# JzHuai0108/sim3opt

Measured on AMD Instinct MI355X. Metric: LM iterations/s, higher is better.
Workload: dtype f64

## Files before the change

include/sim3opt.h:

```cpp
#ifndef SIM3OPT_H
#define SIM3OPT_H

#include <stdint.h>

#ifdef __cplusplus
extern "C" {
#endif

typedef struct sim3opt_graph sim3opt_graph;

enum {
  SIM3OPT_OK = 0,
  SIM3OPT_ERR_ARG = -1,
  SIM3OPT_ERR_STATE = -2,
  SIM3OPT_ERR_NO_DEVICE = -3,
  SIM3OPT_ERR_HIP = -4,
  SIM3OPT_ERR_IO = -5,
  SIM3OPT_ERR_COMM = -6
};

enum { SIM3OPT_KERNEL_NONE = 0, SIM3OPT_KERNEL_HUBER = 1, SIM3OPT_KERNEL_PSEUDO_HUBER = 2,
       SIM3OPT_KERNEL_CAUCHY = 3, SIM3OPT_KERNEL_GEMAN_MCCLURE = 4, SIM3OPT_KERNEL_WELSCH = 5,
       SIM3OPT_KERNEL_FAIR = 6, SIM3OPT_KERNEL_TUKEY = 7, SIM3OPT_KERNEL_SATURATED = 8,
       SIM3OPT_KERNEL_DCS = 9 };

typedef struct sim3opt_options {
  double tau;
  double user_lambda_init;
  double good_step_lower;
  double good_step_upper;
  int32_t max_trials;
  double fd_delta;
  double exp_eps;
  int32_t small_rot_half;
  int32_t fix_small_angle_b;
  int32_t dof_mask;
  int32_t pcg_max_iters;
  double pcg_rel_tol;
  int32_t pcg_check_every;
  int32_t pcg_graph;
  int32_t preconditioner;
  int32_t chain_segment;
  int32_t device;
  int32_t verbose;
  int32_t time_kernels;
  int32_t linear_solver;
  int32_t amg_cycle[4];
  int32_t amg_passes[3];
  int32_t amg_additive;
  int32_t amg_fp32;
  int32_t amg_pivot;
  int32_t amg_coarsest;
  int32_t adaptive_prec;
  int32_t row_order;
  int32_t halo_exchange;
  int32_t span_grid;
  int32_t force_collectives;
  int32_t amg_shard_rows;
  int32_t amg_virtual_ranks;
  int32_t pcg_batch;
  double amg_omega;
  double amg_over[2];
  int64_t direct_max_pairs;
  int32_t debug_full_arrays;
  int32_t jacobians;
  int32_t algorithm;
  int32_t dl_max_trials;
  double dl_delta_init;
  double dl_lambda_init;
  double dl_lambda_factor;
  double cov_workspace_mb;
  int32_t cov_solver;
  double cov_rel_tol;
} sim3opt_options;

enum {
  SIM3OPT_ALGORITHM_LM = 0,
  SIM3OPT_ALGORITHM_GAUSS_NEWTON = 1,
  SIM3OPT_ALGORITHM_DOGLEG = 2
};

enum {
  SIM3OPT_STEP_UNDEFINED = 0,
  SIM3OPT_STEP_SD = 1,
  SIM3OPT_STEP_GN = 2,
  SIM3OPT_STEP_DL = 3
};

typedef struct sim3opt_tr_stats {
  double delta_before;
  double delta_after;
  double alpha;
  double norm_sd;
  double norm_gn;
  double norm_dl;
  int32_t step;
  int32_t was_pd;
} sim3opt_tr_stats;

typedef struct sim3opt_iter_stats {
  double chi2_before;
  double chi2_after;
  double lambda;
  double rho;
  int32_t trials;
  int32_t pcg_iters;
  double pcg_rel_res;
  double ms_linearize;
  double ms_solve;
  double ms_update;
  int32_t pcg_capped;
  int32_t reserved_;
} sim3opt_iter_stats;

typedef struct sim3opt_kernel_times {
  double ms_spmv;      int64_t n_spmv;
  double ms_pcg_vec;   int64_t n_pcg_vec;
  double ms_linearize; int64_t n_linearize;
  double ms_chi2;      int64_t n_chi2;
  double ms_update;    int64_t n_update;
  double ms_replicated_levels; int64_t n_replicated_visits;
  int64_t n_batches; int64_t n_batched_solves;
} sim3opt_kernel_times;

typedef struct sim3opt_comm_times {
  double ms_allreduce;  int64_t n_allreduce;  int64_t bytes_allreduce;
// ... 235 lines not shown
```

sim3opt_amd/csrc/amg_kernels.hpp:

```cpp
#pragma once

__global__ __launch_bounds__(WG) void k_amg_adjoint(int nb, const int32_t* __restrict__ row2v,
                                                    const Sim3* __restrict__ states,
                                                    double* __restrict__ P) {
  for (int i = blockIdx.x * WG + threadIdx.x; i < nb; i += gridDim.x * WG) {
  const Sim3 S = load_sim3(states + row2v[i]);
  double R[9];
  sim3::R_from_quat(S.q, R);
  double A[49];
#pragma unroll
  for (int k = 0; k < 49; ++k) A[k] = 0.0;
  const double t0 = S.t[0], t1 = S.t[1], t2 = S.t[2];
#pragma unroll
  for (int c = 0; c < 3; ++c) {
    const double v0 = R[c], v1 = R[3 + c], v2 = R[6 + c];
    A[0 + 7 * c] = v0;
    A[1 + 7 * c] = v1;
    A[2 + 7 * c] = v2;
    A[3 + 7 * c] = t1 * v2 - t2 * v1;
    A[4 + 7 * c] = t2 * v0 - t0 * v2;
    A[5 + 7 * c] = t0 * v1 - t1 * v0;
    A[3 + 7 * (3 + c)] = S.s * v0;
    A[4 + 7 * (3 + c)] = S.s * v1;
    A[5 + 7 * (3 + c)] = S.s * v2;
// ... 461 lines not shown
  for (int m = 0; m < PB; ++m) {
    double cm[4], rm[4];
#pragma unroll
    for (int a = 0; a < 4; ++a) cm[a] = colk[ty + 16 * a][m];
#pragma unroll
    for (int b = 0; b < 4; ++b) rm[b] = rowk[m][tx + 16 * b];
#pragma unroll
    for (int a = 0; a < 4; ++a)
#pragma unroll
      for (int b = 0; b < 4; ++b) v[a][b] -= cm[a] * rm[b];
  }
#pragma unroll
  for (int a = 0; a < 4; ++a) {
    const int i = i0 + ty + 16 * a, ip = i - k0;
    const bool ik = ip >= 0 && ip < PB;
#pragma unroll
    for (int b = 0; b < 4; ++b) {
      const int jl = tx + 16 * b, j = j0 + jl;
      if (i < n && j < n) B[(size_t)i * n + j] = ik ? rowk[ip][jl] : v[a][b];
    }
  }
}

template <int K>
__global__ __launch_bounds__(WG) void k_amg_dense_apply(int n, const double* __restrict__ Ainv,
                                                        const double* __restrict__ r,
                                                        double* __restrict__ x, int64_t as, int64_t vs) {
  const int lane = threadIdx.x & 63;
  if (gridDim.y > 1) {
    const size_t s0 = (size_t)blockIdx.y * K;
    Ainv += s0 * as;
    r += s0 * vs;
    x += s0 * vs;
  }
  for (int i = blockIdx.x * 4 + (threadIdx.x >> 6); i < n; i += gridDim.x * 4) {
#pragma unroll
    for (int s = 0; s < K; ++s) {
      const double* row = Ainv + (size_t)s * as + (size_t)i * n;
      const double* rs = r + (size_t)s * vs;
      double a0 = 0.0, a1 = 0.0, a2 = 0.0, a3 = 0.0;
      int j = lane;
      for (; j + 192 < n; j += 256) {
        const double m0 = row[j], m1 = row[j + 64], m2 = row[j + 128], m3 = row[j + 192];
        a0 += m0 * rs[j]; a1 += m1 * rs[j + 64]; a2 += m2 * rs[j + 128]; a3 += m3 * rs[j + 192];
      }
      for (; j < n; j += 64) a0 += row[j] * rs[j];
      double acc = (a0 + a1) + (a2 + a3);
      acc = wave_sum(acc);
      if (lane == 0) x[(size_t)s * vs + i] = acc;
    }
  }
}

__global__ __launch_bounds__(WG) void k_to_f32(size_t n, const double* __restrict__ src,
                                               float* __restrict__ dst) {
  for (size_t i = (size_t)blockIdx.x * WG + threadIdx.x; i < n; i += (size_t)gridDim.x * WG)
    dst[f32_pair_index((int64_t)(i / 49), (int)(i % 49))] = (float)src[i];
}
```

sim3opt_amd/csrc/capi.cpp:

```cpp
#include <algorithm>
#include <cmath>
#include <cstdlib>
#include <chrono>
#include <cstring>
#include <memory>
#include <new>
#include <string>
#include <vector>

#include "../../include/sim3opt.h"
#include "../../include/sim3opt_bench.h"
#include "amg.hpp"
#include "col_plan.hpp"
#include "comm.hpp"
#include "devmem.hpp"
#include "direct.hpp"
#include "engine.hpp"
#include "graph.hpp"
#include "robust.hpp"
#include "sim3_jac.hpp"

using namespace sim3opt;

struct sim3opt_graph {
// ... 106 lines not shown

int sim3opt_version(void) { return 130; }

void sim3opt_options_default(sim3opt_options* o) {
  if (!o) return;
  o->tau = 1e-5;
  o->user_lambda_init = 0.0;
  o->good_step_lower = 1.0 / 3.0;
  o->good_step_upper = 2.0 / 3.0;
  o->max_trials = 10;
  o->fd_delta = 1e-9;
  o->exp_eps = 1e-5;
  o->small_rot_half = 0;
  o->fix_small_angle_b = 0;
  o->dof_mask = 127;
  o->pcg_max_iters = 0;
  o->pcg_rel_tol = 1e-10;
  o->pcg_check_every = 16;
  o->pcg_graph = 1;
  o->preconditioner = -1;
  o->chain_segment = 256;
  o->device = -1;
  o->verbose = 0;
  o->time_kernels = 0;
  o->linear_solver = -1;
  for (int32_t& v : o->amg_cycle) v = 0;
  for (int32_t& v : o->amg_passes) v = 0;
  o->amg_additive = 0;
  o->amg_fp32 = 1;
  o->amg_pivot = 14;
  o->amg_coarsest = 256;
  o->adaptive_prec = 1;
  o->row_order = -1;
  o->halo_exchange = 1;
  o->span_grid = 0;
  o->force_collectives = 0;
  o->amg_shard_rows = 4096;
  o->amg_virtual_ranks = 0;
  o->pcg_batch = 0;
  o->amg_omega = 0.9;
  o->amg_over[0] = 1.8;
  o->amg_over[1] = 1.6;
  o->direct_max_pairs = 0;
  o->debug_full_arrays = 0;
  o->jacobians = 0;
  o->algorithm = SIM3OPT_ALGORITHM_LM;
  o->dl_max_trials = 100;
  o->dl_delta_init = 1e4;
  o->dl_lambda_init = 1e-7;
  o->dl_lambda_factor = 10.0;
  o->cov_workspace_mb = 256.0;
  o->cov_solver = 0;
  o->cov_rel_tol = 1e-8;
}

static void apply_env_overrides(sim3opt_options& o) {
  auto digits = [](const char* ev, int32_t* dst, int n, int lo, int hi) {
    int last = 0;
    const int len = (int)std::strlen(ev);
    for (int l = 0; l < n; ++l) {
      if (l < len && ev[l] - '0' >= lo && ev[l] - '0' <= hi) last = ev[l] - '0';
      dst[l] = last;
    }
  };
  if (const char* ev = std::getenv("SIM3OPT_AMG_CYCLE")) digits(ev, o.amg_cycle, 4, 1, 3);
  if (const char* ev = std::getenv("SIM3OPT_AMG_PASSES")) digits(ev, o.amg_passes, 3, 1, 6);
  if (const char* ev = std::getenv("SIM3OPT_AMG_ADDITIVE")) o.amg_additive = std::atoi(ev) != 0;
  if (const char* ev = std::getenv("SIM3OPT_AMG_FP32")) o.amg_fp32 = std::atoi(ev) != 0;
  if (const char* ev = std::getenv("SIM3OPT_AMG_PIVOT")) o.amg_pivot = std::atoi(ev);
  if (const char* ev = std::getenv("SIM3OPT_AMG_COARSEST")) o.amg_coarsest = std::atoi(ev);
  if (const char* ev = std::getenv("SIM3OPT_ADAPTIVE_PREC")) o.adaptive_prec = std::atoi(ev) != 0;
  if (const char* ev = std::getenv("SIM3OPT_ROW_ORDER")) o.row_order = std::string(ev) == "bfs" ? 1 : 0;
  if (std::getenv("SIM3OPT_NO_HALO")) o.halo_exchange = 0;
  if (const char* ev = std::getenv("SIM3OPT_SPAN_GRID")) o.span_grid = std::atoi(ev);
  if (const char* ev = std::getenv("SIM3OPT_FORCE_COMM")) o.force_collectives = ev[0] == '1';
  if (const char* ev = std::getenv("SIM3OPT_AMG_SHARD_ROWS")) o.amg_shard_rows = std::atoi(ev);
  if (const char* ev = std::getenv("SIM3OPT_AMG_VIRTUAL_RANKS")) o.amg_virtual_ranks = std::atoi(ev);
  if (const char* ev = std::getenv("SIM3OPT_PCG_BATCH")) o.pcg_batch = std::atoi(ev);
  if (const char* ev = std::getenv("SIM3OPT_AMG_OMEGA")) o.amg_omega = std::atof(ev);
  if (const char* ev = std::getenv("SIM3OPT_AMG_OVER")) {
    o.amg_over[0] = o.amg_over[1] = std::atof(ev);
    if (const char* c = std::strchr(ev, ',')) o.amg_over[1] = std::atof(c + 1);
  }
  if (const char* ev = std::getenv("SIM3OPT_DIRECT_MAX_PAIRS")) o.direct_max_pairs = std::atoll(ev);
  if (const char* ev = std::getenv("SIM3OPT_DEBUG_FULL_ARRAYS")) o.debug_full_arrays = std::atoi(ev) != 0;
  if (const char* ev = std::getenv("SIM3OPT_COV_WORKSPACE_MB"))
    if (std::atof(ev) > 0.0) o.cov_workspace_mb = std::atof(ev);
  if (const char* ev = std::getenv("SIM3OPT_COV_SOLVER"))
    if (std::atoi(ev) >= 0 && std::atoi(ev) <= 2) o.cov_solver = std::atoi(ev);
  if (const char* ev = std::getenv("SIM3OPT_COV_REL_TOL"))
    if (std::atof(ev) > 0.0 && std::atof(ev) <= 1e-2) o.cov_rel_tol = std::atof(ev);
}

sim3opt_graph* sim3opt_create(void) {
  sim3opt_graph* g = new (std::nothrow) sim3opt_graph();
  if (g) {
    sim3opt_options_default(&g->opt);
    sim3opt::handle_count(+1);
  }
  return g;
}

void sim3opt_destroy(sim3opt_graph* g) {
  if (!g) return;
  delete g;
  if (sim3opt::handle_count(-1) == 0) sim3opt::dev_cache_release();
}

void sim3opt_release_device_cache(void) { sim3opt::dev_cache_release(); }

int sim3opt_set_options(sim3opt_graph* g, const sim3opt_options* o) {
  if (!g || !o) return fail(g, SIM3OPT_ERR_ARG, "set_options: null argument");
  if (!(o->fd_delta > 0) || !(o->exp_eps > 0) || o->max_trials < 1 || !(o->pcg_rel_tol >= 0) ||
      !(o->tau > 0) || o->pcg_check_every < 0 || o->amg_virtual_ranks < 0 || o->pcg_batch < 0 ||
      o->direct_max_pairs < 0 || !(o->amg_omega > 0) || !(o->amg_over[0] > 0) || !(o->amg_over[1] > 0))
    return fail(g, SIM3OPT_ERR_ARG, "set_options: value out of range");
  if (o->jacobians != 0 && o->jacobians != 1)
    return fail(g, SIM3OPT_ERR_ARG, "set_options: jacobians must be 0 (numeric) or 1 (analytic)");
  if (o->algorithm < SIM3OPT_ALGORITHM_LM || o->algorithm > SIM3OPT_ALGORITHM_DOGLEG)
    return fail(g, SIM3OPT_ERR_ARG, "set_options: algorithm must be 0 (LM), 1 (Gauss-Newton) or 2 (dogleg)");
  {
    auto pos = [](double v) { return std::isfinite(v) && v > 0.0; };
// ... 946 lines not shown
```

sim3opt_amd/csrc/engine_amg.hip:

```cpp
#include "engine_impl.hpp"

#include <cassert>

namespace sim3opt {

#include "spmv_kernel.hpp"
#include "amg_kernels.hpp"

int Engine::amg_init(const Structure& s, bool automatic, std::string& err) {
  (void)err;
  amg_omega = std::max(0.1, std::min(0.95, opt.amg_omega));
  amg_additive = opt.amg_additive != 0;
  {
    const bool partitioned = part_world() >= 2;
    int last = 0;
    for (int l = 1; l <= AMG_MAX_LEVELS; ++l) {
      const int o = l <= 4 ? opt.amg_cycle[l - 1] : 0;
      if (o >= 1 && o <= 3) last = o;
      amg_visits[l] = last > 0 ? last : (partitioned ? (l <= 1 ? 1 : 2) : (l <= 1 ? 2 : 3));
    }
    amg_visits[0] = 1;
  }
  amg_fp32 = opt.amg_fp32 != 0;
  adaptive_prec = opt.adaptive_prec != 0 && automatic;
  amg_pivot = opt.amg_pivot >= 28 ? 28 : 14;
  for (int l = 0; l <= AMG_MAX_LEVELS; ++l)
    amg_over_l[l] = std::max(0.5, std::min(3.0, l == 0 ? opt.amg_over[0] : opt.amg_over[1]));
  std::string why;
  AmgBuildOptions bo;
  bo.max_coarsest = opt.amg_coarsest;
  for (int k = 0; k < 3; ++k) bo.passes[k] = opt.amg_passes[k];
  std::vector<int32_t> vbegin;
  bo.world = part_world();
  bo.shard_rows = std::max(1, opt.amg_shard_rows);
  if (comm.world > 1) {
    bo.row_begin = row_begin.data();
  } else if (bo.world > 1) {
    vbegin.resize(bo.world + 1);
    partition_rows_equal(nb, bo.world, vbegin.data());
    bo.row_begin = vbegin.data();
  }
  if (!build_amg_hierarchy(nb, s.rowptr.data(), s.colidx.data(), amg_host, why, bo)) {
    if (opt.verbose) std::fprintf(stderr, "sim3opt: no multigrid hierarchy (%s)\n", why.c_str());
    amg_host.clear();
    return SIM3OPT_OK;
  }
  if (automatic && (double)amg_host[1].nnzb > 0.3 * (double)amg_host[0].nnzb) {
    if (opt.verbose)
      std::fprintf(stderr, "sim3opt: the graph coarsens like an expander (level-1 blocks %.2f of level 0): block-Jacobi\n",
                   (double)amg_host[1].nnzb / (double)amg_host[0].nnzb);
    amg_host.clear();
    return SIM3OPT_OK;
  }
  use_amg = true;
  return SIM3OPT_OK;
}

int Engine::amg_bind(const Structure& s, std::string& err) {
  std::vector<AmgLevelHost>& H = amg_host;
  const int nl = (int)H.size();
  amg.assign(nl, AmgLevel());
  int rc = SIM3OPT_OK;
#define AMGCHK(call) do { rc = (call); if (rc) return rc; } while (0)
  AmgLevel& L0 = amg[0];
  L0.nb = nb; L0.nnzb = nnzb;
  L0.rowptr = d_rowptr; L0.colidx = d_colidx; L0.wrow = d_wrow; L0.span_grid = span_grid;
  L0.vals = d_vals; L0.Minv = d_Minv; L0.r = d_r; L0.x = d_z;
  int64_t padded = 0;
  (void)allgather_equal_plan(offs.data(), comm.world, nullptr, &padded);
  AMGCHK(amg_alloc(d_az, std::max<size_t>((size_t)n, (size_t)padded), err));
  AMGCHK(amg_alloc(d_P, (size_t)49 * nb, err));
  AMGCHK(amg_up(d_row2v, s.row2vertex, err));
  L0.t = d_az;
  L0.lo = r0; L0.hi = r1;
  const int64_t shard_rows = std::max(1, opt.amg_shard_rows);
  rep_level = 1;
  while (rep_level < nl - 1 && H[rep_level].nb > shard_rows && !H[rep_level].row_begin.empty() &&
         H[rep_level].respects_owner)
// ... 159 lines not shown
    const int pb = pivot_rows(k0), pbn = k0 + pb < nd ? pivot_rows(k0 + pb) : 0;
    if (pb == 28)
      hipLaunchKernelGGL((k_amg_dense_gj_step<28>), gt, dim3(WG), 0, stream, nd, k0, (const double*)src,
                         dst, (const double*)pin, pout, pbn, sc);
    else if (pb == 14)
      hipLaunchKernelGGL((k_amg_dense_gj_step<14>), gt, dim3(WG), 0, stream, nd, k0, (const double*)src,
                         dst, (const double*)pin, pout, pbn, sc);
    else
      hipLaunchKernelGGL((k_amg_dense_gj_step<7>), gt, dim3(WG), 0, stream, nd, k0, (const double*)src,
                         dst, (const double*)pin, pout, pbn, sc);
    k0 += pb;
    std::swap(src, dst);
    std::swap(pin, pout);
  }
}

void Engine::spmv_mode(const CycleView& V, int level, int mode, const double* v, double* out, const double* xc) {
  const AmgLevel& L = amg[level];
  const CycleLevel& B = V.lv[level];
  DevScalars* const sc = level == 0 ? V.sc : nullptr;
  double* const rz_part = level == 0 && mode == 2 && !amg_additive ? V.rz_part : nullptr;
  const BatchStrides bs{B.vs, B.ms, level + 1 < (int)amg.size() ? V.lv[level + 1].vs : 0, B.ms, V.part};
#define PASS(CHV, NTV, MODEV, VT, KV, DIAGV, SLICES, VALS)                                                           \
  hipLaunchKernelGGL((k_spmv_span<CHV, NTV, MODEV, VT, KV, DIAGV>), dim3(L.span_grid, SLICES), dim3(WG), 0, stream, \
                     L.nb, L.wrow, L.rowptr, L.colidx, (const VT*)(VALS), v, out, 0.0, rz_part, B.r,                 \
                     const_cast<double*>(xc), sc, (const double*)B.Minv, 1, (const int32_t*)L.agg, amg_over, bs,     \
                     (const float*)B.diag32)
#define PASS_FINE(CHV, VT, KV, VALS) \
  do { if (mode == 1) PASS(CHV, true, 1, VT, KV, false, 1, VALS); else PASS(CHV, true, 2, VT, KV, false, 1, VALS); } while (0)
#define PASS_COARSE(CHV, VT, KV, DIAGV, SLICES, VALS)                 \
  do {                                                                \
    if (mode == 1) PASS(CHV, false, 1, VT, KV, DIAGV, SLICES, VALS);  \
    else if (mode == 3) PASS(CHV, false, 3, VT, KV, DIAGV, SLICES, VALS); \
    else PASS(CHV, false, 2, VT, KV, DIAGV, SLICES, VALS);            \
  } while (0)
  if (!V.batch) {
    if (amg_fp32) {
      if (level == 0) PASS_FINE(SIM3OPT_F32_CH, float, 1, L.vals32); else PASS_COARSE(SIM3OPT_COARSE_CH, float, 1, false, 1, L.vals32);
    } else {
      if (level == 0) PASS_FINE(8, double, 1, L.vals); else PASS_COARSE(8, double, 1, false, 1, L.vals);
    }
  } else if (level == 0) {
    BATCH_DISPATCH(V.nsys, PASS_FINE(SIM3OPT_F32_CH, float, KS, L.vals32));
  } else if (L.nnzb <= b_slice_blocks) {
    PASS_COARSE(8, float, 1, true, V.nsys, L.vals32);
  } else {
    BATCH_DISPATCH(V.nsys, PASS_COARSE(8, float, KS, true, 1, L.vals32));
  }
#undef PASS_COARSE
#undef PASS_FINE
#undef PASS
}

void Engine::amg_restrict(const CycleView& V, int l, const double* t) {
  const AmgLevel& F = amg[l];
  const AmgLevel& Cc = amg[l + 1];
  const CycleLevel &BF = V.lv[l], &BC = V.lv[l + 1];
  const int a0 = Cc.own_lo, a1 = Cc.own_hi;
  const bool gather = comm.active() && sharded(l) && !sharded(l + 1);
  const double* Minv_c = l + 2 < (int)amg.size() ? BC.Minv : nullptr;
  const double* Minv_k = gather ? nullptr : Minv_c;
  if (l == 0)
    BATCH_DISPATCH(V.nsys, hipLaunchKernelGGL((k_amg_restrict0<KS>), dim3(std::max(1, (a1 - a0 + 3) / 4)), dim3(WG), 0,
                       stream, a0, a1, F.mptr, F.mem, d_P, t, BC.r, Minv_k, BC.x, (const DevScalars*)V.sc, BF.vs,
                       BC.vs, BC.ms));
  else
    hipLaunchKernelGGL((k_amg_restrict<1>), dim3(grid_for((a1 - a0 + 8) / 9, 4), V.nsys), dim3(WG), 0, stream, a0, a1,
                       F.mptr, F.mem, t, BC.r, Minv_k, BC.x, BF.vs, BC.vs, BC.ms);
  if (gather) {
    if (amg_status == SIM3OPT_OK) amg_status = comm.allgatherv(BC.r, lvl_offs[l + 1], stream, amg_err);
    if (Minv_c)
      hipLaunchKernelGGL(k_amg_bjapply, dim3(grid_for((Cc.nb + 8) / 9, 4)), dim3(WG), 0, stream, Cc.nb, Minv_c,
                         (const double*)BC.r, BC.x);
  }
}

void Engine::amg_prolong(const CycleView& V, int l, const double* xc, const double* xin, double* xout) {
  const AmgLevel& F = amg[l];
  const DevScalars* scp = l == 0 ? V.sc : nullptr;
  const int64_t vs_f = V.lv[l].vs, vs_c = V.lv[l + 1].vs;
  auto rows = [&](int lo, int hi, const int32_t* list) {
    const int g = grid_for((hi - lo + 8) / 9, 4);
    if (l == 0)
      BATCH_DISPATCH(V.nsys, hipLaunchKernelGGL((k_amg_prolong<true, KS>), dim3(g), dim3(WG), 0, stream, lo, hi, list,
                         F.agg, d_P, xc, xin, xout, scp, amg_over, vs_f, vs_c));
    else
      BATCH_DISPATCH(V.nsys, hipLaunchKernelGGL((k_amg_prolong<false, KS>), dim3(g), dim3(WG), 0, stream, lo, hi, list,
                         F.agg, (const double*)nullptr, xc, xin, xout, scp, amg_over, vs_f, vs_c));
  };
  rows(F.lo, F.hi, nullptr);
  if (comm.active() && sharded(l) && !parts[l].neighbour)
    amg_exchange(l, xout);
  else if (comm.active() && sharded(l) && parts[l].n_recv > 0 && !parts[l].self_test)
    rows(0, parts[l].n_recv, parts[l].d_recv);
}

void Engine::amg_exchange(int l, double* vec) {
  if (!comm.active() || !sharded(l)) return;
  if (amg_status == SIM3OPT_OK) amg_status = exchange_level(l, vec, amg_err);
}

double* Engine::amg_coarse(const CycleView& V, int l) {
  if (opt.time_kernels && l + 1 == rep_level && part_world() > 1 && !V.batch) {
    if (rep_used + 2 > rep_pool.size()) {
      hipEvent_t e0 = nullptr, e1 = nullptr;
      if (event_acquire(&e0) == hipSuccess && event_acquire(&e1) == hipSuccess) {
        rep_pool.push_back(e0);
        rep_pool.push_back(e1);
      }
    }
    if (rep_used + 2 <= rep_pool.size()) {
      (void)hipEventRecord(rep_pool[rep_used], stream);
      double* res = amg_coarse_body(V, l);
      (void)hipEventRecord(rep_pool[rep_used + 1], stream);
      rep_used += 2;
      return res;
    }
  }
  return amg_coarse_body(V, l);
}

double* Engine::amg_coarse_body(const CycleView& V, int l) {
  const int nl = (int)amg.size();
  const AmgLevel& Cc = amg[l + 1];
  const CycleLevel& BC = V.lv[l + 1];
  if (l + 2 == nl) {
    hipLaunchKernelGGL((k_amg_dense_apply<1>), dim3(std::max(1, std::min(256, (7 * Cc.nb + 3) / 4)), V.nsys), dim3(WG),
                       0, stream, 7 * Cc.nb, (const double*)V.Ainv, (const double*)BC.r, BC.x, V.as, BC.vs);
    return BC.x;
  }
  amg_exchange(l + 1, BC.x);
  double* res = amg_cycle(V, l + 1, BC.x, BC.t);
  for (int g = 1; g < amg_visits[l + 1]; ++g) {
    double* oth = res == BC.x ? BC.t : BC.x;
    amg_exchange(l + 1, res);
    spmv_mode(V, l + 1, 2, res, oth);
    amg_exchange(l + 1, oth);
    res = amg_cycle(V, l + 1, oth, res);
  }
  return res;
}

double* Engine::amg_cycle(const CycleView& V, int l, double* cur, double* other) {
  assert(!V.batch || (amg_fp32 && !amg_additive && !comm.active()));
  spmv_mode(V, l, 1, cur, other);
  amg_restrict(V, l, other);
  double* xc = amg_coarse(V, l);
  amg_exchange(l + 1, xc);
  amg_over = amg_over_on ? amg_over_l[l] : 1.0;
  if (l == 0) {
    amg_prolong(V, l, xc, cur, cur);
    spmv_mode(V, l, 2, cur, other);
  } else {
    spmv_mode(V, l, 3, cur, other, xc);
  }
  return other;
}

int Engine::amg_apply(std::string& err) {
  amg_status = SIM3OPT_OK;
  if (amg_additive) {
    amg_restrict(cv_one, 0, d_r);
    double* xc0 = amg_coarse(cv_one, 0);
    amg_exchange(1, xc0);
    amg_over = amg_over_on ? amg_over_l[0] : 1.0;
    amg_prolong(cv_one, 0, xc0, d_z, d_az);
  } else {
    amg_exchange(0, d_z);
    amg_cycle(cv_one, 0, d_z, d_az);
  }
  if (amg_status == SIM3OPT_OK) amg_exchange(0, d_az);
  if (amg_status != SIM3OPT_OK) {
    err = amg_err;
    return amg_status;
  }
  return SIM3OPT_OK;
}

int Engine::amg_numbers(double lambda, std::string& err) {
// ... 78 lines not shown
```

sim3opt_amd/csrc/engine_impl.hpp:

```cpp
#pragma once
#include <hip/hip_runtime.h>
#include <hip/hip_ext.h>

#include <algorithm>
#include <cfloat>
#include <chrono>
#include <cmath>
#include <cstdio>
#include <cstddef>
#include <cstdlib>
#include <cstring>

#include "amg.hpp"
#include "comm.hpp"
#include "devmem.hpp"
#include "direct_factor.hpp"
#include "engine.hpp"

namespace sim3opt {

using sim3::Sim3;

#define HIPCHK(call)                                                        \
  do {                                                                      \
// ... 123 lines not shown
    T* p = nullptr;
    if (opt.debug_full_arrays) {
      HIPCHK(dev_malloc((void**)&p, sizeof(T) * (size_t)total));
      HIPCHK(hipMemset(p, 0xFF, sizeof(T) * (size_t)total));
      if (hi > lo) HIPCHK(hipMemset(p + lo, 0, sizeof(T) * (size_t)(hi - lo)));
      virt = p;
    } else {
      HIPCHK(dev_malloc((void**)&p, sizeof(T) * (size_t)std::max<int64_t>(hi - lo, 1)));
      HIPCHK(hipMemset(p, 0, sizeof(T) * (size_t)std::max<int64_t>(hi - lo, 1)));
      virt = reinterpret_cast<T*>(reinterpret_cast<uintptr_t>(p) - sizeof(T) * (size_t)lo);
    }
    ranged.push_back({p, sizeof(T), total, lo, hi});
    return SIM3OPT_OK;
  }
  int check_foreign_ranges(std::string& err);
  int64_t ranged_bytes() const {
    int64_t b = 0;
    for (const RangedArray& a : ranged) b += (int64_t)a.elem * (opt.debug_full_arrays ? a.total : std::max<int64_t>(a.hi - a.lo, 1));
    return b;
  }
  double *d_x = nullptr, *d_r = nullptr, *d_z = nullptr, *d_p = nullptr, *d_q = nullptr, *d_s = nullptr;
  double *d_part_a = nullptr, *d_part_b = nullptr;
  int32_t *d_sub_first = nullptr, *d_sub_cnt = nullptr;
  double* d_Gm = nullptr;
  bool use_chain = false;
  int chain_seg = 256;
  struct AmgLevel {
    int32_t nb = 0;
    int64_t nnzb = 0;
    int32_t *rowptr = nullptr, *colidx = nullptr, *wrow = nullptr;
    int span_grid = 0;
    double *vals = nullptr, *diagH = nullptr, *W = nullptr, *Minv = nullptr;
    float* vals32 = nullptr;
    int32_t *agg = nullptr, *mptr = nullptr, *mem = nullptr, *gptr = nullptr, *gblk = nullptr, *grow = nullptr;
    double *r = nullptr, *x = nullptr, *t = nullptr;
    int32_t lo = 0, hi = 0;
    int32_t own_lo = 0, own_hi = 0;
    int64_t own_b0 = 0, own_b1 = 0;
  };
  std::vector<std::vector<int64_t>> lvl_offs, lvl_blk_offs;
  std::vector<AmgLevel> amg;
  std::vector<void*> amg_owned;
  double *d_P = nullptr, *d_Ainv = nullptr, *d_Ainv2 = nullptr, *d_piv = nullptr, *d_az = nullptr;
  int32_t* d_row2v = nullptr;
  bool use_amg = false, amg_stale = true;
  double amg_omega = 0.9;
  int amg_visits[AMG_MAX_LEVELS + 1];
  bool amg_additive = false;
  bool amg_fp32 = true;
  double amg_over_l[AMG_MAX_LEVELS + 1];
  double amg_over = 1.0;
  bool amg_over_on = true;
  int amg_pivot = 14;
  bool adaptive_prec = true;
  double bj_gate = -1.0;
  int bj_budget = 48;
  int n_bj_solves = 0, n_bj_abandoned = 0;
  bool trace_stale = true;
  double mean_diag = 0.0;
  int amg_status = 0;
  std::string amg_err;
  struct CycleLevel {
    double *Minv = nullptr, *r = nullptr, *x = nullptr, *t = nullptr;
    float* diag32 = nullptr;
    int64_t vs = 0, ms = 0;
  };
  struct CycleView {
    int nsys = 1;
    bool batch = false;
    std::vector<CycleLevel> lv;
    DevScalars* sc = nullptr;
    double* Ainv = nullptr;
    int64_t as = 0;
    double* rz_part = nullptr;
    int part = 0;
  };
  CycleView cv_one;
  CycleView cv_batch;
  struct PcgView {
    int nsys = 1;
    int nsc = 1;
    bool batch = false;
    double *x = nullptr, *r = nullptr, *z = nullptr, *p = nullptr, *q = nullptr, *s = nullptr, *az = nullptr;
    int64_t vs = 0;
    double* Minv = nullptr;
    int64_t ms = 0;
    const double* b = nullptr;
    int64_t bstride = 0;
    double tol[KB] = {0, 0, 0, 0}, lam[KB] = {0, 0, 0, 0};
    DevScalars *sc = nullptr, *h_sc = nullptr;
    double *part_a = nullptr, *part_b = nullptr;
    int pstride = 0;
    CycleView* cv = nullptr;
  };
  PcgView pv_one;
  PcgView pv_batch;
  std::vector<void*> batch_owned;
  double *b_x = nullptr, *b_r = nullptr, *b_z = nullptr, *b_p = nullptr, *b_q = nullptr, *b_s = nullptr, *b_az = nullptr;
  double *b_Ainv = nullptr, *b_diag64 = nullptr, *b_part_a = nullptr, *b_part_b = nullptr;
  int64_t b_vs = 0, b_as = 0;
  DevScalars *d_bsc = nullptr, *h_bsc = nullptr;
  bool batch_ready = false;
  int64_t b_slice_blocks = 100000;
  int batch_alloc(std::string& err);
  void batch_release();
  void batch_prepare(int nsetup);
// ... 71 lines not shown

  int init(const HostGraph& g, const Structure& s, std::string& err);

  int fetch_scalars(std::string& err) { return fetch_scalars(pv_one, err); }
  int fetch_scalars(PcgView& V, std::string& err);

  DevScalars* h_ring = nullptr;
  hipEvent_t ring_ev = nullptr;
  static constexpr int sched_cap_mg = 8;
  static constexpr double sched_frac = 0.85;
  int sched_chunk(double rem, int fixed, int cap) const {
    if (rem < 0.0) return fixed;
    return std::max(1, std::min(cap, (int)std::floor(sched_frac * rem)));
  }
  int sched_ahead(double left, int cap) const {
    const int c = std::min(cap, (int)std::floor(0.5 * left));
    return c >= 2 ? c : 0;
  }
  int poll_async(const DevScalars* src, int nsc, std::string& err);
  int poll_wait(DevScalars* dst, int nsc, std::string& err);
  int64_t sched_stats[4] = {0, 0, 0, 0};

  int phase_ms(int a, int b, double& acc, std::string& err);
  int pool_get(hipEvent_t& a, hipEvent_t& b, std::string& err);
  long long spmv_work_seen = 0;
  int pool_drain(std::string& err);

  template <typename T>
  int amg_up(T*& dptr, const std::vector<T>& h, std::string& err) {
    HIPCHK(dev_malloc((void**)&dptr, sizeof(T) * std::max<size_t>(h.size(), 1)));
    amg_owned.push_back(dptr);
    if (!h.empty()) HIPCHK(staged.put(dptr, h.data(), sizeof(T) * h.size(), stream));
    return SIM3OPT_OK;
  }
  int amg_alloc(double*& dptr, size_t count, std::string& err) {
    HIPCHK(dev_malloc((void**)&dptr, sizeof(double) * std::max<size_t>(count, 1)));
    amg_owned.push_back(dptr);
    HIPCHK(hipMemset(dptr, 0, sizeof(double) * std::max<size_t>(count, 1)));
    return SIM3OPT_OK;
  }

  std::vector<AmgLevelHost> amg_host;
  int amg_init(const Structure& s, bool automatic, std::string& err);

  int amg_bind(const Structure& s, std::string& err);

  int amg_setup(std::string& err);

  void amg_prepare(double lambda);

  void spmv_mode(const CycleView& V, int level, int mode, const double* v, double* out, const double* xc = nullptr);

  void amg_restrict(const CycleView& V, int l, const double* t);
  void amg_prolong(const CycleView& V, int l, const double* xc, const double* xin, double* xout);

  double* amg_coarse(const CycleView& V, int l);
  double* amg_coarse_body(const CycleView& V, int l);
  void amg_exchange(int l, double* vec);

  double* amg_cycle(const CycleView& V, int l, double* cur, double* other);

  int amg_apply(std::string& err);

  int direct_init(const Structure& s, std::string& err);

  int direct_solve(double lambda, std::string& err);

  BlockLdl marg_factor;
  std::vector<int32_t> mpos;
  std::string marg_refused;
  int marginal_init(std::string& err);
  int marginals(double lambda, int32_t n, const int32_t* row_a, const int32_t* row_b, double* cov,
                std::string& err);
  int cov_blocks(const char* who, bool any_pair, bool fixed_zero, double lambda, int32_t n, const int32_t* row_a,
                 const int32_t* row_b, double* cov, std::string& err);
  int64_t cov_stats[6] = {0, 0, 0, 0, 0, 0};
  int gate_edges(double lambda, int32_t n, const int32_t* v0, const int32_t* v1, const int32_t* row0,
                 const int32_t* row1, const Sim3* meas, const double* infoinv, double* e_out, double* S_out,
                 double* d2_out, std::string& err);
  std::vector<void*> cols_owned;
  double *c_g = nullptr, *c_y = nullptr, *c_r = nullptr, *c_d = nullptr;
  double* c_nrm = nullptr;
  int64_t c_vs = 0;
  int cols_alloc(std::string& err);
  void cols_release();
  int cols_batch_width() const {
    if (!use_amg || amg.empty() || comm.active() || !amg_fp32 || amg_additive) return 0;
    return opt.pcg_batch >= 1 ? std::min(opt.pcg_batch, KB) : KB;
  }
  int cols_solve(double lambda, int nsys, const double* g, const double* tol, bool setup, const double** x,
                 int32_t* iters, bool* failed, std::string& err);
  int cols_true_residuals(double lambda, int cnt, const int* sys, double* rel, std::string& err);
  int inverse_columns(double lambda, int32_t nvert, const int32_t* vertices, const int32_t* first,
                      const int32_t* blk_row, double* blocks, std::string& err);
  int cov_blocks_columns(const std::string& pre, bool fixed_zero, double lambda, int32_t n, const int32_t* row_a,
                         const int32_t* row_b, double* cov, std::string& err);
  int64_t col_counts[5] = {0, 0, 0, 0, 0};
  double col_res[2] = {0.0, 0.0};
  int32_t col_fail_vertex = -1;
  void jacobi(int lo, int hi, const int32_t* rowptr, double* vals, double lambda, double* Minv, double omega,
              const double* diagH, const double* W, float* vals32, DevScalars* sc = nullptr,
              double* diag64_out = nullptr, float* diag32_out = nullptr);
  void norms2(const double* r, const double* b, double* part_a, double* part_b, double* out2);
  void dense_inverse(const double* diag64, double* Aout, DevScalars* sc);

  int exchange_rows(double* vec, std::string& err) { return exchange_level(0, vec, err); }
// ... 61 lines not shown
```

sim3opt_amd/lib.py:

```python
import ctypes as C
import os
import sys

import numpy as np

_HERE = os.path.dirname(os.path.abspath(__file__))
LIB_PATH = os.environ.get("SIM3OPT_LIB") or os.path.join(_HERE, "libsim3opt.so")

OK, ERR_ARG, ERR_STATE, ERR_NO_DEVICE, ERR_HIP, ERR_IO, ERR_COMM = 0, -1, -2, -3, -4, -5, -6
(KERNEL_NONE, KERNEL_HUBER, KERNEL_PSEUDO_HUBER, KERNEL_CAUCHY, KERNEL_GEMAN_MCCLURE, KERNEL_WELSCH, KERNEL_FAIR,
 KERNEL_TUKEY, KERNEL_SATURATED, KERNEL_DCS) = range(10)
KERNEL_NAMES = ("none", "huber", "pseudo_huber", "cauchy", "geman_mcclure", "welsch", "fair", "tukey", "saturated",
                "dcs")
ALGORITHM_LM, ALGORITHM_GAUSS_NEWTON, ALGORITHM_DOGLEG = 0, 1, 2
STEP_UNDEFINED, STEP_SD, STEP_GN, STEP_DL = 0, 1, 2, 3
STEP_NAMES = ("undefined", "SD", "GN", "DL")


class Options(C.Structure):
    _fields_ = [
        ("tau", C.c_double),
        ("user_lambda_init", C.c_double),
        ("good_step_lower", C.c_double),
        ("good_step_upper", C.c_double),
        ("max_trials", C.c_int32),
        ("fd_delta", C.c_double),
        ("exp_eps", C.c_double),
        ("small_rot_half", C.c_int32),
        ("fix_small_angle_b", C.c_int32),
        ("dof_mask", C.c_int32),
        ("pcg_max_iters", C.c_int32),
        ("pcg_rel_tol", C.c_double),
        ("pcg_check_every", C.c_int32),
        ("pcg_graph", C.c_int32),
        ("preconditioner", C.c_int32),
        ("chain_segment", C.c_int32),
        ("device", C.c_int32),
        ("verbose", C.c_int32),
        ("time_kernels", C.c_int32),
        ("linear_solver", C.c_int32),
        ("amg_cycle", C.c_int32 * 4),
        ("amg_passes", C.c_int32 * 3),
        ("amg_additive", C.c_int32),
        ("amg_fp32", C.c_int32),
        ("amg_pivot", C.c_int32),
        ("amg_coarsest", C.c_int32),
        ("adaptive_prec", C.c_int32),
        ("row_order", C.c_int32),
        ("halo_exchange", C.c_int32),
        ("span_grid", C.c_int32),
        ("force_collectives", C.c_int32),
        ("amg_shard_rows", C.c_int32),
        ("amg_virtual_ranks", C.c_int32),
        ("pcg_batch", C.c_int32),
        ("amg_omega", C.c_double),
        ("amg_over", C.c_double * 2),
        ("direct_max_pairs", C.c_int64),
        ("debug_full_arrays", C.c_int32),
        ("jacobians", C.c_int32),
        ("algorithm", C.c_int32),
        ("dl_max_trials", C.c_int32),
        ("dl_delta_init", C.c_double),
        ("dl_lambda_init", C.c_double),
        ("dl_lambda_factor", C.c_double),
        ("cov_workspace_mb", C.c_double),
        ("cov_solver", C.c_int32),
        ("cov_rel_tol", C.c_double),
    ]


class IterStats(C.Structure):
    _fields_ = [
        ("chi2_before", C.c_double),
        ("chi2_after", C.c_double),
        ("lambda_", C.c_double),
        ("rho", C.c_double),
        ("trials", C.c_int32),
        ("pcg_iters", C.c_int32),
        ("pcg_rel_res", C.c_double),
        ("ms_linearize", C.c_double),
        ("ms_solve", C.c_double),
        ("ms_update", C.c_double),
        ("pcg_capped", C.c_int32),
        ("reserved_", C.c_int32),
    ]


class TrustRegionStats(C.Structure):
    _fields_ = [
        ("delta_before", C.c_double),
        ("delta_after", C.c_double),
        ("alpha", C.c_double),
        ("norm_sd", C.c_double),
        ("norm_gn", C.c_double),
        ("norm_dl", C.c_double),
        ("step", C.c_int32),
        ("was_pd", C.c_int32),
    ]


class BaOptions(C.Structure):
    _fields_ = [
        ("huber_delta", C.c_double),
        ("pixel_noise", C.c_double),
        ("tau", C.c_double),
        ("user_lambda_init", C.c_double),
        ("max_trials", C.c_int32),
        ("pcg_max_iters", C.c_int32),
        ("pcg_rel_tol", C.c_double),
        ("linear_solver", C.c_int32),
        ("device", C.c_int32),
        ("verbose", C.c_int32),
    ]


class BaBatchOptions(C.Structure):
    _fields_ = [
        ("huber_delta", C.c_double),
        ("pixel_noise", C.c_double),
        ("tau", C.c_double),
# ... 1162 lines not shown
```

Baseline: 50.94.

## Fuse coarsest-level AMG restriction with dense inverse apply in one kernel

Adds a kernel that restricts the fine residual into the coarsest-level residual, keeps it in shared memory, and immediately multiplies by the dense inverse, replacing a separate restrict launch and dense-apply launch. Every workgroup recomputes the full restriction redundantly so that no grid-wide synchronisation or global round trip is needed. It is gated on the last two levels being unsharded and the coarse vector fitting in 48 KB of LDS, and is enabled by default with an option to turn it off. The cost is redundant gather work in each block and more LDS and register use per block.

```diff
diff --git a/include/sim3opt.h b/include/sim3opt.h
--- a/include/sim3opt.h
+++ b/include/sim3opt.h
@@ -72,6 +72,7 @@
   double cov_workspace_mb;
   int32_t cov_solver;
   double cov_rel_tol;
+  int32_t amg_fused;
 } sim3opt_options;
 
 enum {
diff --git a/sim3opt_amd/csrc/amg_kernels.hpp b/sim3opt_amd/csrc/amg_kernels.hpp
--- a/sim3opt_amd/csrc/amg_kernels.hpp
+++ b/sim3opt_amd/csrc/amg_kernels.hpp
@@ -537,6 +537,142 @@
   }
 }
 
+constexpr int RD_WG = 512;
+constexpr int RD_MAXQ = AMG_DENSE_MAX_N / 64;
+constexpr int RD_SLOTS = 2;
+constexpr int RD_CHUNK = 4;
+static_assert(AMG_DENSE_MAX_N % 64 == 0, "a lane holds RD_MAXQ entries of a row of the dense inverse");
+static_assert(4 * AMG_MAX_COARSEST <= RD_WG * RD_SLOTS, "a workgroup forms all of r_c in one sweep");
+typedef double rd_pair __attribute__((ext_vector_type(2), aligned(8)));
+template <int K>
+__global__ __launch_bounds__(RD_WG) void k_amg_restrict_dense(int nc, const int32_t* __restrict__ mptr,
+                                                              const int32_t* __restrict__ mem,
+                                                              const double* __restrict__ t_f,
+                                                              double* __restrict__ r_c,
+                                                              const double* __restrict__ Ainv,
+                                                              double* __restrict__ x_c, int64_t vs_f, int64_t vs_c,
+                                                              int64_t as) {
+  extern __shared__ double rd_rc[];
+  const int n = 7 * nc;
+  const int tid = threadIdx.x, lane = tid & 63, wave = tid >> 6;
+  if (gridDim.y > 1) {
+    const size_t s0 = (size_t)blockIdx.y * K;
+    t_f += s0 * vs_f;
+    r_c += s0 * vs_c;
+    x_c += s0 * vs_c;
+    Ainv += s0 * as;
+  }
+  int i = blockIdx.x * (RD_WG / 64) + wave;
+  double m[RD_MAXQ];
+  auto load_row = [&](int row, int s) {
+    const double* p = Ainv + (size_t)s * as + (size_t)row * n;
+#pragma unroll
+    for (int q = 0; q < RD_MAXQ; ++q) {
+      const int j = lane + 64 * q;
+      m[q] = p[j < n ? j : 0];
+    }
+  };
+  load_row(i < n ? i : 0, 0);
+  {
+    int e0[RD_SLOTS], cnt[RD_SLOTS], ecl[RD_SLOTS], off[RD_SLOTS], mi[RD_SLOTS][RD_CHUNK];
+    int maxcnt = 0;
+#pragma unroll
+    for (int p = 0; p < RD_SLOTS; ++p) {
+      const int idx = tid + RD_WG * p;
+      const bool act = idx < 4 * nc;
+      const int a = act ? idx >> 2 : 0, h = idx & 3;
+      off[p] = h < 3 ? 2 * h : 5;
+      e0[p] = mptr[a];
+      cnt[p] = act ? mptr[a + 1] - e0[p] : 0;
+      ecl[p] = cnt[p] > 0 ? e0[p] + cnt[p] - 1 : (e0[p] > 0 ? e0[p] - 1 : 0);
+      maxcnt = cnt[p] > maxcnt ? cnt[p] : maxcnt;
+    }
+#pragma unroll
+    for (int p = 0; p < RD_SLOTS; ++p)
+#pragma unroll
+      for (int q = 0; q < RD_CHUNK; ++q) mi[p][q] = mem[q < cnt[p] ? e0[p] + q : ecl[p]];
+    rd_pair acc[RD_SLOTS][K];
+#pragma unroll
+    for (int p = 0; p < RD_SLOTS; ++p)
+#pragma unroll
+      for (int s = 0; s < K; ++s) acc[p][s] = rd_pair{0.0, 0.0};
+    for (int b = 0; b < maxcnt; b += RD_CHUNK) {
+      int mn[RD_SLOTS][RD_CHUNK];
+#pragma unroll
+      for (int p = 0; p < RD_SLOTS; ++p)
+#pragma unroll
+        for (int q = 0; q < RD_CHUNK; ++q)
+          mn[p][q] = mem[b + RD_CHUNK + q < cnt[p] ? e0[p] + b + RD_CHUNK + q : ecl[p]];
+#pragma unroll
+      for (int s = 0; s < K; ++s) {
+        const double* tf = t_f + (size_t)s * vs_f;
+        rd_pair v[RD_SLOTS][RD_CHUNK];
+#pragma unroll
+        for (int p = 0; p < RD_SLOTS; ++p)
+#pragma unroll
+          for (int q = 0; q < RD_CHUNK; ++q) v[p][q] = *(const rd_pair*)(tf + (size_t)7 * mi[p][q] + off[p]);
+#pragma unroll
+        for (int p = 0; p < RD_SLOTS; ++p) {
+          const int ng = cnt[p] >> 2;
+          static_assert(RD_CHUNK == 4, "a chunk is one group of four, or the singles behind the last group");
+          const rd_pair grp = (v[p][0] + v[p][1]) + (v[p][2] + v[p][3]);
+          acc[p][s] = b / 4 < ng ? acc[p][s] + grp : acc[p][s];
+#pragma unroll
+          for (int q = 0; q < RD_CHUNK; ++q) acc[p][s] = b + q >= 4 * ng && b + q < cnt[p] ? acc[p][s] + v[p][q] : acc[p][s];
+        }
+      }
+#pragma unroll
+      for (int p = 0; p < RD_SLOTS; ++p)
+#pragma unroll
+        for (int q = 0; q < RD_CHUNK; ++q) mi[p][q] = mn[p][q];
+    }
+#pragma unroll
+    for (int p = 0; p < RD_SLOTS; ++p) {
+      const int idx = tid + RD_WG * p;
+      if (idx < 4 * nc) {
+        const int a = idx >> 2, h = idx & 3;
+#pragma unroll
+        for (int s = 0; s < K; ++s) {
+          double* out = rd_rc + s * n + 7 * a;
+          if (h < 3) out[2 * h] = acc[p][s].x;
+          out[h < 3 ? 2 * h + 1 : 6] = acc[p][s].y;
+          if (blockIdx.x == 0) {
+            double* g = r_c + (size_t)s * vs_c + 7 * a;
+            if (h < 3) g[2 * h] = acc[p][s].x;
+            g[h < 3 ? 2 * h + 1 : 6] = acc[p][s].y;
+          }
+        }
+      }
+    }
+  }
+  __syncthreads();
+  bool have = true;
+  for (; i < n; i += gridDim.x * (RD_WG / 64)) {
+#pragma unroll
+    for (int s = 0; s < K; ++s) {
+      if (!have) load_row(i, s);
+      have = false;
+      const double* rs = rd_rc + s * n;
+      double a0 = 0.0, a1 = 0.0, a2 = 0.0, a3 = 0.0;
+#pragma unroll
+      for (int g = 0; g < RD_MAXQ / 4; ++g) {
+        const int j = lane + 256 * g;
+        if (j + 192 < n) {
+          a0 += m[4 * g] * rs[j]; a1 += m[4 * g + 1] * rs[j + 64];
+          a2 += m[4 * g + 2] * rs[j + 128]; a3 += m[4 * g + 3] * rs[j + 192];
+        } else {
+#pragma unroll
+          for (int u = 0; u < 3; ++u)
+            if (j + 64 * u < n) a0 += m[4 * g + u] * rs[j + 64 * u];
+        }
+      }
+      double acc = (a0 + a1) + (a2 + a3);
+      acc = wave_sum(acc);
+      if (lane == 0) x_c[(size_t)s * vs_c + i] = acc;
+    }
+  }
+}
+
 __global__ __launch_bounds__(WG) void k_to_f32(size_t n, const double* __restrict__ src,
                                                float* __restrict__ dst) {
   for (size_t i = (size_t)blockIdx.x * WG + threadIdx.x; i < n; i += (size_t)gridDim.x * WG)
diff --git a/sim3opt_amd/csrc/capi.cpp b/sim3opt_amd/csrc/capi.cpp
--- a/sim3opt_amd/csrc/capi.cpp
+++ b/sim3opt_amd/csrc/capi.cpp
@@ -182,6 +182,7 @@
   o->cov_workspace_mb = 256.0;
   o->cov_solver = 0;
   o->cov_rel_tol = 1e-8;
+  o->amg_fused = 1;
 }
 
 static void apply_env_overrides(sim3opt_options& o) {
@@ -198,6 +199,7 @@
   if (const char* ev = std::getenv("SIM3OPT_AMG_ADDITIVE")) o.amg_additive = std::atoi(ev) != 0;
   if (const char* ev = std::getenv("SIM3OPT_AMG_FP32")) o.amg_fp32 = std::atoi(ev) != 0;
   if (const char* ev = std::getenv("SIM3OPT_AMG_PIVOT")) o.amg_pivot = std::atoi(ev);
+  if (const char* ev = std::getenv("SIM3OPT_AMG_FUSED")) o.amg_fused = std::atoi(ev) != 0;
   if (const char* ev = std::getenv("SIM3OPT_AMG_COARSEST")) o.amg_coarsest = std::atoi(ev);
   if (const char* ev = std::getenv("SIM3OPT_ADAPTIVE_PREC")) o.adaptive_prec = std::atoi(ev) != 0;
   if (const char* ev = std::getenv("SIM3OPT_ROW_ORDER")) o.row_order = std::string(ev) == "bfs" ? 1 : 0;
diff --git a/sim3opt_amd/csrc/engine_amg.hip b/sim3opt_amd/csrc/engine_amg.hip
--- a/sim3opt_amd/csrc/engine_amg.hip
+++ b/sim3opt_amd/csrc/engine_amg.hip
@@ -24,6 +24,7 @@
   amg_fp32 = opt.amg_fp32 != 0;
   adaptive_prec = opt.adaptive_prec != 0 && automatic;
   amg_pivot = opt.amg_pivot >= 28 ? 28 : 14;
+  amg_fused = opt.amg_fused != 0;
   for (int l = 0; l <= AMG_MAX_LEVELS; ++l)
     amg_over_l[l] = std::max(0.5, std::min(3.0, l == 0 ? opt.amg_over[0] : opt.amg_over[1]));
   std::string why;
@@ -289,10 +290,23 @@
 #undef PASS
 }
 
+bool Engine::amg_restrict_solves(int l) const {
+  const bool gather = comm.active() && sharded(l) && !sharded(l + 1);
+  return amg_fused && l >= 1 && l + 2 == (int)amg.size() && !gather &&
+         sizeof(double) * 7 * (size_t)amg[l + 1].nb <= 48 * 1024;
+}
+
 void Engine::amg_restrict(const CycleView& V, int l, const double* t) {
   const AmgLevel& F = amg[l];
   const AmgLevel& Cc = amg[l + 1];
   const CycleLevel &BF = V.lv[l], &BC = V.lv[l + 1];
+  if (amg_restrict_solves(l)) {
+    const int nd = 7 * Cc.nb, rows = RD_WG / 64;
+    hipLaunchKernelGGL((k_amg_restrict_dense<1>), dim3((nd + rows - 1) / rows, V.nsys), dim3(RD_WG),
+                       sizeof(double) * nd, stream, Cc.nb, F.mptr, F.mem, t, BC.r, (const double*)V.Ainv, BC.x, BF.vs,
+                       BC.vs, V.as);
+    return;
+  }
   const int a0 = Cc.own_lo, a1 = Cc.own_hi;
   const bool gather = comm.active() && sharded(l) && !sharded(l + 1);
   const double* Minv_c = l + 2 < (int)amg.size() ? BC.Minv : nullptr;
@@ -362,6 +376,7 @@
   const AmgLevel& Cc = amg[l + 1];
   const CycleLevel& BC = V.lv[l + 1];
   if (l + 2 == nl) {
+    if (amg_restrict_solves(l)) return BC.x;
     hipLaunchKernelGGL((k_amg_dense_apply<1>), dim3(std::max(1, std::min(256, (7 * Cc.nb + 3) / 4)), V.nsys), dim3(WG),
                        0, stream, 7 * Cc.nb, (const double*)V.Ainv, (const double*)BC.r, BC.x, V.as, BC.vs);
     return BC.x;
diff --git a/sim3opt_amd/csrc/engine_impl.hpp b/sim3opt_amd/csrc/engine_impl.hpp
--- a/sim3opt_amd/csrc/engine_impl.hpp
+++ b/sim3opt_amd/csrc/engine_impl.hpp
@@ -199,6 +199,7 @@
   double amg_over = 1.0;
   bool amg_over_on = true;
   int amg_pivot = 14;
+  bool amg_fused = true;
   bool adaptive_prec = true;
   double bj_gate = -1.0;
   int bj_budget = 48;
@@ -376,6 +377,7 @@
   void spmv_mode(const CycleView& V, int level, int mode, const double* v, double* out, const double* xc = nullptr);
 
   void amg_restrict(const CycleView& V, int l, const double* t);
+  bool amg_restrict_solves(int l) const;
   void amg_prolong(const CycleView& V, int l, const double* xc, const double* xin, double* xout);
 
   double* amg_coarse(const CycleView& V, int l);
diff --git a/sim3opt_amd/lib.py b/sim3opt_amd/lib.py
--- a/sim3opt_amd/lib.py
+++ b/sim3opt_amd/lib.py
@@ -66,6 +66,7 @@
         ("cov_workspace_mb", C.c_double),
         ("cov_solver", C.c_int32),
         ("cov_rel_tol", C.c_double),
+        ("amg_fused", C.c_int32),
     ]
 
 
```

Measured after the change: 49.49. 0.971x the previous value.
